# ferdean/lsa-fw

Measured on AMD Instinct MI355X. Metric: converged eigenpairs/sec (k=20, shift-invert), higher is better.
Workload: dtype c128

## Files before the change

lsa-fw_amd/csrc/ndlu.hip:

```cpp
#include <algorithm>
#include <chrono>
#include <cmath>
#include <cstdlib>
#include <functional>
#include <new>
#include <string>

#include "lsa_internal.h"
#include "nd_internal.h"

int k_allgather_inplace(lsa_ctx* ctx, void* vec, size_t bytes_per_rank);

namespace {

constexpr int kRT = 32;
constexpr int kCH = 1024;
constexpr int kGT = 64;

inline double now_s() { return std::chrono::duration<double>(std::chrono::steady_clock::now().time_since_epoch()).count(); }
inline size_t esize(int dtype) { return dtype == LSA_C128 ? 16 : 8; }

struct NdNodeDev {
    int64_t front_off;
    int64_t lfac_off;
// ... 1070 lines not shown
    for (int32_t c0 = 0; c0 < b; c0 += kCH) {
        const int32_t cn = min(kCH, b - c0);
        for (int32_t j = tid; j < cn; j += 256) vs[j] = bv[c0 + j];
        __syncthreads();
        if (c0 == 0) two_row_dot_prefetched<LPR>(Ua, Ub, vs, cn, sl, acc0, acc1, pa, pb);
        else two_row_dot<LPR>(Ua + c0, Ub + c0, vs, cn, sl, acc0, acc1);
        __syncthreads();
    }
    acc0 = lanes_sum<LPR>(acc0);
    acc1 = lanes_sum<LPR>(acc1);
    if (sl == 0) {
        if (ra < m) {
            const VT v = s_sub(xa, acc0);
            x[ia] = v;
            push_down(ge, nd.nchild, f, ra, xb, v);
        }
        if (rb < m) {
            const VT v = s_sub(xc, acc1);
            x[ib] = v;
            push_down(ge, nd.nchild, f, rb, xb, v);
        }
    }
    if (nd.nchild > 0) {
        const int32_t ntile = (m + ROWS - 1) / ROWS;
        const int64_t total = (int64_t)nd.nchild * b;
        for (int64_t e = (int64_t)ty * 256 + tid; e < total; e += (int64_t)ntile * 256) {
            const int32_t c = (int32_t)(e / b), j = (int32_t)(e - (int64_t)c * b);
            const int32_t g = ge[(size_t)c * f + m + j];
            if (g >= 0) xb[g] = bv[j];
        }
    }
}

template <typename MT, typename VT, int LPR, bool ORDERED>
__global__ __launch_bounds__(256) void nd_bwd_kernel(const NdSweepNode* __restrict__ lnodes, const MT* __restrict__ ufac,
                                                     const int32_t* __restrict__ idx, const int32_t* __restrict__ gell, VT* __restrict__ x,
                                                     VT* __restrict__ xb) {
    __shared__ VT vs[kCH];
    const NdSweepNode nd = lnodes[blockIdx.x];
    const int32_t r0 = (int32_t)blockIdx.y * (512 / LPR);
    if (r0 >= nd.m || nd.f == nd.m) return;
    nd_bwd_tile<MT, VT, LPR, ORDERED>(nd, r0, (int32_t)blockIdx.y, vs, ufac, idx, gell, x, xb);
}

constexpr int kNdBatchMax = 16;
struct NdBatchPtrs {
    const void* lfac[kNdBatchMax];
    const void* ufac[kNdBatchMax];
    const void* rhs[kNdBatchMax];
    void* x[kNdBatchMax];
    void* ubuf[kNdBatchMax];
    void* acc[kNdBatchMax];
    void* xb[kNdBatchMax];
};

template <typename MT, typename VT, int LPR, bool ORDERED>
__global__ __launch_bounds__(256) void nd_fwd_batch_kernel(const NdSweepNode* __restrict__ lnodes, const int32_t* __restrict__ idx,
                                                           const int32_t* __restrict__ gell, const int32_t* __restrict__ cmap, NdBatchPtrs p) {
    __shared__ VT vs[kCH];
    const NdSweepNode nd = lnodes[blockIdx.x];
    const int32_t r0 = (int32_t)blockIdx.y * (512 / LPR);
    if (r0 >= nd.orows + nd.brow) return;
    const int z = blockIdx.z;
    nd_fwd_tile<MT, VT, LPR, ORDERED>(nd, r0, vs, (const MT*)p.lfac[z], idx, gell, cmap, (const VT*)p.rhs[z], (VT*)p.x[z], (VT*)p.ubuf[z], (VT*)p.acc[z],
                                      (VT*)p.xb[z]);
}

template <typename MT, typename VT, int LPR, bool ORDERED>
__global__ __launch_bounds__(256) void nd_bwd_batch_kernel(const NdSweepNode* __restrict__ lnodes, const int32_t* __restrict__ idx,
                                                           const int32_t* __restrict__ gell, NdBatchPtrs p) {
    __shared__ VT vs[kCH];
    const NdSweepNode nd = lnodes[blockIdx.x];
    const int32_t r0 = (int32_t)blockIdx.y * (512 / LPR);
    if (r0 >= nd.m || nd.f == nd.m) return;
    const int z = blockIdx.z;
    nd_bwd_tile<MT, VT, LPR, ORDERED>(nd, r0, (int32_t)blockIdx.y, vs, (const MT*)p.ufac[z], idx, gell, (VT*)p.x[z], (VT*)p.xb[z]);
}

template <typename VT, bool ORDERED>
__global__ __launch_bounds__(256) void nd_dist_pack_kernel(const int32_t* __restrict__ dnodes, const NdNodeDev* __restrict__ nodes,
                                                           const int32_t* __restrict__ idx, int32_t rank, const VT* __restrict__ x, VT* __restrict__ xg) {
    const NdNodeDev nd = nodes[dnodes[blockIdx.x]];
    const int32_t r = (int32_t)blockIdx.y * 256 + threadIdx.x;
    if (r >= nd.orows) return;
    const int32_t j = nd.orow0 + r;
    xg[nd.xg_base + (int64_t)rank * nd.xg_stride + r] = x[ORDERED ? nd.own0 + j : idx[nd.idx_off + j]];
}

template <typename VT, bool ORDERED>
__global__ __launch_bounds__(256) void nd_dist_unpack_kernel(const int32_t* __restrict__ dnodes, const NdNodeDev* __restrict__ nodes,
                                                             const int32_t* __restrict__ child_ptr, const int32_t* __restrict__ child_idx,
                                                             const int32_t* __restrict__ cmap, const int32_t* __restrict__ idx, int32_t nranks,
                                                             VT* x, const VT* __restrict__ xg, VT* xb) {
    const int32_t t = dnodes[blockIdx.x];
    const NdNodeDev nd = nodes[t];
    const int32_t m = nd.m, b = nd.f - m;
    const int32_t ms = (m + nranks - 1) / nranks;
    const int32_t i = (int32_t)blockIdx.z * 256 + threadIdx.x;
    (void)b;
    auto own_val = [&](int32_t j) -> VT { return xg[nd.xg_base + (int64_t)(j / ms) * nd.xg_stride + j % ms]; };
    if (blockIdx.y == 0) {
        if (i >= m) return;
        x[ORDERED ? nd.own0 + i : idx[nd.idx_off + i]] = own_val(i);
        return;
    }
    const int32_t cp = child_ptr[t] + (int32_t)blockIdx.y - 1;
    if (cp >= child_ptr[t + 1]) return;
    const NdNodeDev nc = nodes[child_idx[cp]];
    if (i >= nc.f - nc.m) return;
    const int32_t p = cmap[nc.cmap_off + i];
    xb[nc.u_off + i] = p < m ? own_val(p) : xb[nd.u_off + (p - m)];
}

template <bool CONJ, typename MT>
__device__ __forceinline__ MT maybe_conj(MT a) {
    if constexpr (CONJ) return s_conj(a);
    else return a;
}

template <typename MT, typename VT, bool CONJ, bool DOWN>
__global__ __launch_bounds__(256) void nd_sweepT_kernel(const NdSweepNode* __restrict__ lnodes, const MT* __restrict__ lfac, const MT* __restrict__ ufac,
                                                        const int32_t* __restrict__ idx, const int32_t* __restrict__ gell,
                                                        const VT* __restrict__ rhs, VT* __restrict__ x, VT* __restrict__ ubuf,
                                                        const int64_t* __restrict__ tgoff, VT* __restrict__ pz, int64_t tg_slot, int32_t rank) {
    __shared__ VT vs[kCH];
    __shared__ VT part[4][64];
    const NdSweepNode nd = lnodes[blockIdx.x];
    const int32_t m = nd.m, f = nd.f, b = f - m;
    const bool dist = (nd.flags & 1) != 0;
// ... 62 lines not shown
        x[ix[r]] = s_add(x[ix[r]], z);
    } else if (r < m) {
        x[ix[r]] = z;
    } else {
        const int32_t j = r - m, w = (b + nranks - 1) / nranks, owner = j / w;
        const VT u = s_sub(gather_updates(gell + nd.ge_off, nd.nchild, f, r, ubuf, scalar_traits<VT>::zero()), z);
        ubuf[nd.u_off + (int64_t)(owner - rank) * ux_slot + (j - owner * w)] = u;
    }
}

}

struct lsa_ndlu {
    lsa_ctx* ctx = nullptr;
    NdSymbolic S;
    int dtype = LSA_C128;
    bool ordered = false;
    std::vector<NdChunk> chunks;
    std::vector<NdLevel> levels;
    NdNodeDev* d_nodes = nullptr;
    NdSweepNode *d_lnodes = nullptr, *d_lnodes_bwd = nullptr;
    int32_t *d_dist_nodes = nullptr, *d_child_ptr = nullptr, *d_child_idx = nullptr;
    void *d_xstage = nullptr, *d_xg = nullptr;
    int64_t* d_tgoff = nullptr;
    void* d_tg = nullptr;
    std::vector<int64_t> tg_slot;
    int64_t tg_slot_max = 0;
    int64_t xstage_slot = 0;
    std::vector<int64_t> h_upd_off, h_lfac_off;
    int64_t chunk_node_upd_off(int32_t t) const { return h_upd_off[(size_t)t]; }
    int32_t* d_gell = nullptr;
    int32_t *d_idx = nullptr, *d_cmap = nullptr, *d_tiles = nullptr, *d_chunk_nodes = nullptr;
    int64_t* d_asm_dst = nullptr;
    int32_t* d_asm_src = nullptr;
    int64_t asm_count = 0;
    int32_t *d_ipiv = nullptr, *d_rowq = nullptr, *d_flag = nullptr, *d_xflag = nullptr;
    unsigned long long* d_maxabs = nullptr;
    void *d_lfac = nullptr, *d_ufac = nullptr;
    void *d_work = nullptr, *d_upd = nullptr;
    void *d_ubuf = nullptr, *d_xb = nullptr, *d_acc = nullptr;
    void *d_tmp = nullptr, *d_ybuf = nullptr;
    int64_t lfac_entries = 0, ufac_entries = 0, work_entries = 0, upd_entries = 0, acc_entries = 0;
    int64_t xupd_slot = 0;
    int32_t *d_cand[2] = {nullptr, nullptr};
    void* d_dinv = nullptr;
    int32_t tp_min = 1 << 30;
    int32_t sb_min = 1 << 30;
    int32_t sb_cols = 128;
    int32_t ycap = 32;
    hipStream_t side = nullptr;
    hipEvent_t ev_panel = nullptr, ev_pivots = nullptr;
    double seconds_analyse = 0.0, seconds_numeric = 0.0;
    int32_t solve_launches = 0;
    int acc_vbytes = 0;
};

namespace {

void nd_free(lsa_ndlu* f) {
    if (!f) return;
    for (void* p : {(void*)f->d_lnodes_bwd, (void*)f->d_dist_nodes, (void*)f->d_child_ptr, (void*)f->d_child_idx, f->d_xstage, f->d_xg, (void*)f->d_tgoff, f->d_tg})
        if (p) (void)hipFree(p);
    for (void* p : {(void*)f->d_nodes, (void*)f->d_lnodes, (void*)f->d_gell, (void*)f->d_idx, (void*)f->d_cmap, (void*)f->d_tiles,
                    (void*)f->d_chunk_nodes, (void*)f->d_asm_dst, (void*)f->d_asm_src, (void*)f->d_ipiv, (void*)f->d_rowq, (void*)f->d_flag, (void*)f->d_xflag, (void*)f->d_maxabs,
                    f->d_lfac, f->d_ufac, f->d_work, f->d_upd, f->d_ubuf, f->d_xb, f->d_acc, f->d_tmp, f->d_ybuf, (void*)f->d_cand[0], (void*)f->d_cand[1], f->d_dinv})
        if (p) (void)hipFree(p);
    if (f->ev_panel) (void)hipEventDestroy(f->ev_panel);
    if (f->ev_pivots) (void)hipEventDestroy(f->ev_pivots);
    if (f->side) (void)hipStreamDestroy(f->side);
    delete f;
}

template <typename U>
int upload(lsa_ctx* ctx, const std::vector<U>& h, U** d) {
    const size_t bytes = std::max<size_t>(h.size(), 1) * sizeof(U);
    LSA_HIP_ALLOC(ctx, hipMalloc((void**)d, bytes));
    if (!h.empty()) LSA_HIP_CHECK(ctx, hipMemcpy(*d, h.data(), h.size() * sizeof(U), hipMemcpyHostToDevice));
    return LSA_OK;
}

int nd_setup(lsa_ctx* ctx, lsa_ndlu* f, int64_t free_agreed = 0) {
    NdSymbolic& S = f->S;
    const int32_t nt = S.nt;
    const size_t es = esize(f->dtype);
    const bool dist = S.nranks > 1;
    {
        const char* e = getenv("LSA_ND_TP_MIN");
        f->tp_min = e && *e ? std::max(1, atoi(e)) : 512;
        const char* sbm = getenv("LSA_ND_SB_MIN");
        f->sb_min = std::max(f->tp_min, sbm && *sbm ? std::max(1, atoi(sbm)) : 1024);
        f->ycap = kNB;
        const char* sbc = getenv("LSA_ND_SB_COLS");
        f->sb_cols = sbc && *sbc ? std::min(1024, std::max(kGT, atoi(sbc) / kGT * kGT)) : kSB;
    }
    LSA_HIP_ALLOC(ctx, hipMalloc((void**)&f->d_xflag, 4 * sizeof(int32_t) * (size_t)std::max(1, S.nranks)));
    f->ordered = true;
    for (size_t k = 0; k < S.perm.size() && f->ordered; ++k) f->ordered = S.perm[k] == (int32_t)k || dist;
    if (dist)
        for (int32_t t = 0; t < nt && f->ordered; ++t)
            for (int32_t r = 1; r < S.m[(size_t)t]; ++r)
                if (S.idx[(size_t)S.idx_off[(size_t)t] + r] != S.idx[(size_t)S.idx_off[(size_t)t]] + r) {
                    f->ordered = false;
                    break;
                }
    std::vector<NdNodeDev> nodes((size_t)nt);
    std::vector<int32_t> tiles;
    auto begin_list = [&](TileList& tl) { tl.off = (int64_t)tiles.size() / 2; tl.count = 0; };
    auto push = [&](TileList& tl, int32_t a, int32_t b) {
        tiles.push_back(a);
        tiles.push_back(b);
        ++tl.count;
    };
    int64_t budget = 0;
    {
        size_t free_b = 0, total_b = 0;
        if (hipMemGetInfo(&free_b, &total_b) != hipSuccess) free_b = (size_t)16 << 30;
        const int64_t after = (int64_t)free_b - S.factor_entries * (int64_t)es;
        budget = std::max<int64_t>(after / 4, (int64_t)256 << 20) / (int64_t)es;
        if (S.has_dist) budget = std::max<int64_t>((free_agreed > 0 ? free_agreed : (int64_t)free_b) / 6, (int64_t)256 << 20) / (int64_t)es;
        if (const char* e = getenv("LSA_ND_WORK_MB")) budget = std::max<int64_t>(atoll(e), 1) * (1 << 20) / (int64_t)es;
    }
    if (getenv("LSA_ND_TEST_OOM"))
        return lsa_set_error(ctx, LSA_ERR_OOM, "lsa_ndlu: out of device memory (forced by LSA_ND_TEST_OOM)");
    NdMemoryPlan P;
    nd_memory_plan(S, budget, P);
    for (int32_t t = 0; t < nt; ++t) {
        NdNodeDev& nd = nodes[(size_t)t];
        nd.front_off = P.work_off[(size_t)t];
        nd.lfac_off = P.lfac_off[(size_t)t];
        nd.ufac_off = P.ufac_off[(size_t)t];
// ... 236 lines not shown
                for (int32_t cp = S.child_ptr[(size_t)t]; cp < S.child_ptr[(size_t)t + 1]; ++cp) {
                    const int32_t ch = S.child_idx[(size_t)cp];
                    L.dist_rows = std::max(L.dist_rows, S.f[(size_t)ch] - S.m[(size_t)ch]);
                }
            }
        }
        LSA_CHECK(upload(ctx, lnodes, &f->d_lnodes));
        LSA_CHECK(upload(ctx, bnodes, &f->d_lnodes_bwd));
        LSA_CHECK(upload(ctx, dist_nodes, &f->d_dist_nodes));
        LSA_CHECK(upload(ctx, S.child_ptr, &f->d_child_ptr));
        LSA_CHECK(upload(ctx, S.child_idx, &f->d_child_idx));
        if (f->xstage_slot > 0) LSA_HIP_ALLOC(ctx, hipMalloc(&f->d_xstage, (size_t)f->xstage_slot * (size_t)S.nranks * es));
        if (S.xg_entries > 0) LSA_HIP_ALLOC(ctx, hipMalloc(&f->d_xg, (size_t)S.xg_entries * 16));
    }
    LSA_CHECK(upload(ctx, S.gell, &f->d_gell));
    LSA_CHECK(upload(ctx, S.idx, &f->d_idx));
    LSA_CHECK(upload(ctx, S.cmap, &f->d_cmap));
    LSA_CHECK(upload(ctx, chunk_nodes, &f->d_chunk_nodes));
    LSA_CHECK(upload(ctx, tiles, &f->d_tiles));
    const size_t nn = (size_t)std::max<int32_t>(S.n, 1);
    LSA_HIP_ALLOC(ctx, hipMalloc((void**)&f->d_ipiv, nn * sizeof(int32_t)));
    LSA_HIP_ALLOC(ctx, hipMalloc((void**)&f->d_rowq, nn * sizeof(int32_t)));
    LSA_HIP_ALLOC(ctx, hipMalloc((void**)&f->d_flag, 4 * sizeof(int32_t)));
    LSA_HIP_ALLOC(ctx, hipMalloc((void**)&f->d_maxabs, sizeof(unsigned long long)));
    LSA_HIP_ALLOC(ctx, hipMalloc(&f->d_lfac, (size_t)std::max<int64_t>(f->lfac_entries, 1) * es));
    LSA_HIP_ALLOC(ctx, hipMalloc(&f->d_ufac, (size_t)std::max<int64_t>(f->ufac_entries, 1) * es));
    LSA_HIP_ALLOC(ctx, hipMalloc(&f->d_work, (size_t)f->work_entries * es));
    LSA_HIP_ALLOC(ctx, hipMalloc(&f->d_upd, (size_t)f->upd_entries * es));
    const size_t ub = (size_t)std::max<int64_t>(S.u_off[(size_t)nt], 1) * 16;
    LSA_HIP_ALLOC(ctx, hipMalloc(&f->d_ubuf, ub));
    LSA_HIP_ALLOC(ctx, hipMalloc(&f->d_xb, ub));
    LSA_HIP_ALLOC(ctx, hipMalloc(&f->d_acc, (size_t)std::max<int64_t>(f->acc_entries, 1) * 16));
    LSA_HIP_CHECK(ctx, hipMemsetAsync(f->d_acc, 0, (size_t)std::max<int64_t>(f->acc_entries, 1) * 16, ctx->stream));
    LSA_HIP_CHECK(ctx, hipMemsetAsync(f->d_ubuf, 0, ub, ctx->stream));
    LSA_HIP_CHECK(ctx, hipMemsetAsync(f->d_xb, 0, ub, ctx->stream));
    LSA_HIP_ALLOC(ctx, hipMalloc(&f->d_tmp, nn * 16));
    LSA_HIP_ALLOC(ctx, hipMalloc(&f->d_ybuf, nn * (size_t)f->ycap * es));
    if (widest_tp > 0) {
        const size_t cand = ((size_t)S.n / kTRmin + (size_t)nt + 1) * kNB * sizeof(int32_t);
        LSA_HIP_ALLOC(ctx, hipMalloc((void**)&f->d_cand[0], cand));
        LSA_HIP_ALLOC(ctx, hipMalloc((void**)&f->d_cand[1], cand));
        LSA_HIP_ALLOC(ctx, hipMalloc(&f->d_dinv, (size_t)widest_tp * kNB * kNB * es));
        const char* la = getenv("LSA_ND_LOOKAHEAD");
        if (!(la && *la && atoi(la) == 0)) {
            int lo_pri = 0, hi_pri = 0;
            LSA_HIP_CHECK(ctx, hipDeviceGetStreamPriorityRange(&lo_pri, &hi_pri));
            LSA_HIP_CHECK(ctx, hipStreamCreateWithPriority(&f->side, hipStreamNonBlocking, hi_pri));
            LSA_HIP_CHECK(ctx, hipEventCreateWithFlags(&f->ev_panel, hipEventDisableTiming));
            LSA_HIP_CHECK(ctx, hipEventCreateWithFlags(&f->ev_pivots, hipEventDisableTiming));
        }
    }
    f->solve_launches = 0;
    for (const NdLevel& L : f->levels) f->solve_launches += (L.fwd_tiles > 0) + (L.bwd_tiles > 0);
    return LSA_OK;
}

template <typename T, int NT, int RPT, int W>
void launch_block(lsa_ctx* ctx, lsa_ndlu* f, const NdChunk& L, int32_t kb, double tiny2) {
    hipStream_t st = ctx->stream;
    const int32_t* lv = f->d_chunk_nodes + L.node_begin;
    T* front = (T*)f->d_work;
    auto active_at = [&](int32_t k) {
        return (int32_t)(std::lower_bound(L.sorted_m.begin(), L.sorted_m.end(), k, std::greater<int32_t>()) - L.sorted_m.begin());
    };
    const int32_t kend = std::min(kb + kNB, L.max_m);
    const bool others = std::min(kNB, L.max_m - kb) > W;
    int32_t kprev = -1, active_prev = 0;
    for (int32_t k0 = kb; k0 < kend; k0 += W) {
        const int32_t active = active_at(k0);
        if (active == 0) break;
        hipLaunchKernelGGL((nd_gj_fused_kernel<T, NT, RPT, W>), dim3(std::max(active, active_prev), others && kprev >= 0 ? 1 + kNB / 16 : 1), dim3(NT), 0, st, lv,
                           f->d_nodes, front, f->d_ipiv, f->d_rowq, kb, k0, kprev, f->d_flag, tiny2);
        kprev = k0;
        active_prev = active;
    }
    if (others && kprev >= 0)
        hipLaunchKernelGGL((nd_gj_fused_kernel<T, NT, RPT, W>), dim3(active_prev, 1 + kNB / 16), dim3(NT), 0, st, lv, f->d_nodes, front, f->d_ipiv, f->d_rowq, kb,
                           -1, kprev, f->d_flag, tiny2);
    if (L.max_m > kNB) {
        const int32_t active = active_at(kb);
        hipLaunchKernelGGL((nd_gj_stage_kernel<T>), dim3(active, (L.max_m + 255) / 256), dim3(256), 0, st, lv, f->d_nodes, (const T*)front, f->d_ipiv, kb,
                           kNB, kNB, 0, L.max_m, (T*)f->d_ybuf);
        const int32_t tiles = (L.max_m + kGT - 1) / kGT;
        hipLaunchKernelGGL((nd_gj_gemm_kernel<T>), dim3(active, tiles, tiles), dim3(256), 0, st, lv, f->d_nodes, front, f->d_rowq, kb, (const T*)f->d_ybuf, 0, 0,
                           0, 0, 0);
    }
}

template <typename T>
void launch_tournament(lsa_ndlu* f, const NdChunk& L, int32_t kb, double tiny2, hipStream_t st) {
    const int32_t* lv = f->d_chunk_nodes + L.node_begin;
    const T* front = (const T*)f->d_work;
    const int32_t active = (int32_t)(std::lower_bound(L.sorted_m.begin(), L.sorted_m.end(), kb, std::greater<int32_t>()) - L.sorted_m.begin());
    if (active == 0) return;
    int32_t sets = (L.max_m + tp_first<T>::rows - 1) / tp_first<T>::rows;
    hipLaunchKernelGGL((nd_tp_round_kernel<T, true, false>), dim3(active, sets), dim3(256), 0, st, lv, f->d_nodes, front, f->d_ipiv, f->d_rowq, kb, 0,
                       (const int32_t*)nullptr, f->d_cand[0], (T*)nullptr, f->d_flag, tiny2);
    int src = 0;
    for (int32_t round = 0;; ++round) {
        const int32_t groups = (sets + kTA - 1) / kTA;
        if (groups == 1) {
            hipLaunchKernelGGL((nd_tp_round_kernel<T, false, true>), dim3(active, 1), dim3(256), 0, st, lv, f->d_nodes, front, f->d_ipiv, f->d_rowq, kb, round,
                               (const int32_t*)f->d_cand[src], (int32_t*)nullptr, (T*)f->d_dinv, f->d_flag, tiny2);
            break;
        }
        hipLaunchKernelGGL((nd_tp_round_kernel<T, false, false>), dim3(active, groups), dim3(256), 0, st, lv, f->d_nodes, front, f->d_ipiv, f->d_rowq, kb, round,
// ... 106 lines not shown
        }
        for (const TileList& e : L.ext)
            if (e.count > 0)
                hipLaunchKernelGGL((nd_extend_add_kernel<T>), dim3(e.count), dim3(256), 0, st, tl + 2 * e.off, f->d_nodes, f->d_cmap, front, (const T*)upd);
        for (const auto& step : L.xsteps) {
            T* stage = (T*)f->d_xstage;
            int64_t stride = 0;
            for (int r = 0; r < S.nranks; ++r) {
                const NdChunk::XPiece& pc = step[(size_t)r];
                if (pc.nrows > 0) stride = std::max(stride, (int64_t)pc.nrows * (S.f[(size_t)pc.child] - S.m[(size_t)pc.child]));
            }
            if (stride == 0) continue;
            const NdChunk::XPiece& mine = step[(size_t)S.rank];
            if (mine.nrows > 0) {
                const int32_t bc = S.f[(size_t)mine.child] - S.m[(size_t)mine.child];
                const int64_t src_off = f->chunk_node_upd_off(mine.child) + (int64_t)(mine.row0 - S.brow0[(size_t)mine.child]) * bc;
                LSA_HIP_CHECK(ctx, hipMemcpyAsync(stage + (size_t)S.rank * (size_t)stride, upd + src_off, (size_t)mine.nrows * (size_t)bc * sizeof(T),
                                                  hipMemcpyDeviceToDevice, st));
            }
            LSA_CHECK(k_allgather_inplace(ctx, stage, (size_t)stride * sizeof(T)));
            for (int r = 0; r < S.nranks; ++r) {
                const NdChunk::XPiece& pc = step[(size_t)r];
                if (pc.nrows <= 0) continue;
                hipLaunchKernelGGL((nd_extend_add_staged_kernel<T>), dim3((pc.nrows + 15) / 16), dim3(256), 0, st, f->d_nodes, f->d_cmap, front,
                                   (const T*)(stage + (size_t)r * (size_t)stride), pc.child, pc.row0, pc.nrows);
            }
        }
        if (L.max_m >= f->tp_min) LSA_CHECK(launch_level_tp<T>(ctx, f, L, tiny2));
        for (int32_t kb = 0; kb < L.max_m && L.max_m < f->tp_min; kb += kNB) {
            if (L.max_m <= 64) launch_block<T, 64, 1, 8>(ctx, f, L, kb, tiny2);
            else if (L.max_m <= 128) launch_block<T, 128, 1, 8>(ctx, f, L, kb, tiny2);
            else if (L.max_m <= 256) launch_block<T, 256, 1, 8>(ctx, f, L, kb, tiny2);
            else if (L.max_m <= 512) launch_block<T, 512, 1, 8>(ctx, f, L, kb, tiny2);
            else if (L.max_m <= 1024) launch_block<T, 1024, 1, 8>(ctx, f, L, kb, tiny2);
            else if (L.max_m <= 2048) launch_block<T, 1024, 2, 8>(ctx, f, L, kb, tiny2);
            else if (L.max_m <= 4096) launch_block<T, 1024, 4, 4>(ctx, f, L, kb, tiny2);
            else if (L.max_m <= 8192) launch_block<T, 1024, 8, 2>(ctx, f, L, kb, tiny2);
            else launch_block<T, 1024, 16, 1>(ctx, f, L, kb, tiny2);
        }
        if (L.unperm.count > 0)
            hipLaunchKernelGGL((nd_unperm_kernel<T>), dim3(L.unperm.count), dim3(256), 0, st, tl + 2 * L.unperm.off, f->d_nodes, front, f->d_ipiv,
                               f->d_rowq, lfac);
        auto product = [&](auto kind) {
            constexpr int KIND = decltype(kind)::value;
            if (L.gemm[KIND].count == 0) return;
            hipLaunchKernelGGL((nd_gemm_mfma_kernel<T, KIND>), dim3(L.gemm[KIND].count), dim3(256), 0, st, tl + 2 * L.gemm[KIND].off, f->d_nodes, front, lfac, ufac);
        };
        product(std::integral_constant<int, 0>{});
        product(std::integral_constant<int, 1>{});
        product(std::integral_constant<int, 2>{});
        if (L.save.count > 0)
            hipLaunchKernelGGL((nd_save_update_kernel<T>), dim3(L.save.count), dim3(256), 0, st, tl + 2 * L.save.off, f->d_nodes, (const T*)front, upd);
    }
    if (!exchanged && S.nranks > 1 && f->xupd_slot > 0)
        LSA_CHECK(k_allgather_inplace(ctx, f->d_upd, (size_t)f->xupd_slot * sizeof(T)));
    int32_t hflag[4] = {0, 0, 0, 0};
    if (S.nranks > 1) {
        LSA_HIP_CHECK(ctx, hipMemcpyAsync(f->d_xflag + 4 * S.rank, f->d_flag, 4 * sizeof(int32_t), hipMemcpyDeviceToDevice, st));
        LSA_CHECK(k_allgather_inplace(ctx, f->d_xflag, 4 * sizeof(int32_t)));
        std::vector<int32_t> all((size_t)4 * S.nranks, 0);
        LSA_HIP_CHECK(ctx, hipMemcpyAsync(all.data(), f->d_xflag, all.size() * sizeof(int32_t), hipMemcpyDeviceToHost, st));
        LSA_HIP_CHECK(ctx, hipStreamSynchronize(st));
        for (int r = 0; r < S.nranks; ++r)
            if (all[(size_t)4 * r + 1] != 0) {
                memcpy(hflag, &all[(size_t)4 * r], sizeof hflag);
                if (r != S.rank) hflag[1] = -(r + 1);
                break;
            }
    } else {
        LSA_HIP_CHECK(ctx, hipMemcpyAsync(hflag, f->d_flag, sizeof hflag, hipMemcpyDeviceToHost, st));
        LSA_HIP_CHECK(ctx, hipStreamSynchronize(st));
    }
    LSA_HIP_CHECK(ctx, hipGetLastError());
    if (hflag[1] < 0)
        return lsa_set_error(ctx, LSA_ERR_ZERO_PIVOT, "lsa_ndlu: a pivot block on rank %d is singular to 1e-15 * max|C| (column %d of its node)", -hflag[1] - 1,
                             hflag[2]);
    if (hflag[1] != 0) {
        const int32_t t = hflag[1] - 1;
        const unsigned long long hi = (unsigned long long)(uint32_t)hflag[3] << 32;
        double mag2;
        memcpy(&mag2, &hi, sizeof mag2);
        return lsa_set_error(ctx, LSA_ERR_ZERO_PIVOT,
                             "lsa_ndlu: the pivot block of tree node %d (%d unknowns, front %d, level %d) is singular at its column %d: largest "
                             "candidate pivot %.3e against max|C| = %.3e (threshold 1e-15 max|C|); the matrix is singular, or needs pivoting "
                             "across fronts",
                             t, S.m[(size_t)t], S.f[(size_t)t], S.level[(size_t)t], hflag[2], std::sqrt(mag2), std::sqrt(max2));
    }
    if (const char* pe = getenv("LSA_ND_TEST_PERTURB")) {
        const double eps = atof(pe);
        if (eps != 0.0 && f->ufac_entries > 0) {
            const int blocks = (int)std::min<int64_t>((f->ufac_entries + 255) / 256, (int64_t)ctx->num_cu * 16);
            hipLaunchKernelGGL((nd_scale_kernel<T>), dim3(blocks), dim3(256), 0, st, f->ufac_entries, ufac, 1.0 + eps);
            LSA_HIP_CHECK(ctx, hipStreamSynchronize(st));
        }
    }
    return LSA_OK;
}

template <typename MT, typename VT, bool ORDERED>
int nd_apply_ordered(lsa_ctx* ctx, lsa_ndlu* f, const VT* b, VT* x) {
    hipStream_t st = ctx->stream;
    const MT* lfac = (const MT*)f->d_lfac;
    const MT* ufac = (const MT*)f->d_ufac;
    const NdSymbolic& S = f->S;
    VT *ubuf = (VT*)f->d_ubuf, *acc = (VT*)f->d_acc, *xb = (VT*)f->d_xb;
    if (f->acc_vbytes != (int)sizeof(VT)) {
        LSA_HIP_CHECK(ctx, hipMemsetAsync(f->d_acc, 0, (size_t)std::max<int64_t>(f->acc_entries, 1) * 16, st));
        f->acc_vbytes = (int)sizeof(VT);
    }
    for (size_t li = 0; li <= f->levels.size(); ++li) {
        if ((int32_t)li == S.phase_b_level && S.nranks > 1 && S.xu_slot > 0) LSA_CHECK(k_allgather_inplace(ctx, f->d_ubuf, (size_t)S.xu_slot * sizeof(VT)));
        if (li == f->levels.size()) break;
        const NdLevel& L = f->levels[li];
        if (L.fwd_tiles > 0) {
            const dim3 grid(L.node_count, L.fwd_tiles);
            const NdSweepNode* ln = f->d_lnodes + L.node_begin;
            if (L.sweep_rows == 8)
                hipLaunchKernelGGL((nd_fwd_kernel<MT, VT, 64, ORDERED>), grid, dim3(256), 0, st, ln, lfac, f->d_idx, f->d_gell, f->d_cmap, b, x, ubuf, acc, xb);
            else if (L.sweep_rows == 128)
                hipLaunchKernelGGL((nd_fwd_kernel<MT, VT, 4, ORDERED>), grid, dim3(256), 0, st, ln, lfac, f->d_idx, f->d_gell, f->d_cmap, b, x, ubuf, acc, xb);
            else
                hipLaunchKernelGGL((nd_fwd_kernel<MT, VT, 16, ORDERED>), grid, dim3(256), 0, st, ln, lfac, f->d_idx, f->d_gell, f->d_cmap, b, x, ubuf, acc, xb);
        }
        if (L.dist_count > 0 && L.ux_slot > 0) LSA_CHECK(k_allgather_inplace(ctx, ubuf + L.ux_base, (size_t)L.ux_slot * sizeof(VT)));
    }
    for (size_t l = f->levels.size(); l-- > 0;) {
        const NdLevel& L = f->levels[l];
        if (L.bwd_tiles > 0) {
            const dim3 grid(L.node_count, L.bwd_tiles);
            const NdSweepNode* ln = f->d_lnodes_bwd + L.node_begin;
            if (L.sweep_rows == 8) hipLaunchKernelGGL((nd_bwd_kernel<MT, VT, 64, ORDERED>), grid, dim3(256), 0, st, ln, ufac, f->d_idx, f->d_gell, x, xb);
            else hipLaunchKernelGGL((nd_bwd_kernel<MT, VT, 16, ORDERED>), grid, dim3(256), 0, st, ln, ufac, f->d_idx, f->d_gell, x, xb);
        }
        if (L.dist_count > 0) {
            const int32_t* dn = f->d_dist_nodes + L.dist_begin;
            VT* xg = (VT*)f->d_xg;
            if (L.xg_slot > 0) {
                hipLaunchKernelGGL((nd_dist_pack_kernel<VT, ORDERED>), dim3(L.dist_count, (L.dist_rows + 255) / 256), dim3(256), 0, st, dn, f->d_nodes, f->d_idx, S.rank,
                                   (const VT*)x, xg);
                LSA_CHECK(k_allgather_inplace(ctx, xg + L.xg_base, (size_t)L.xg_slot * sizeof(VT)));
            }
            hipLaunchKernelGGL((nd_dist_unpack_kernel<VT, ORDERED>), dim3(L.dist_count, 1 + L.dist_children, (L.dist_rows + 255) / 256), dim3(256), 0, st, dn, f->d_nodes,
                               f->d_child_ptr, f->d_child_idx, f->d_cmap, f->d_idx, S.nranks, x, (const VT*)xg, xb);
        }
    }
    LSA_HIP_CHECK(ctx, hipGetLastError());
    return LSA_OK;
}

template <typename MT, typename VT>
int nd_apply(lsa_ctx* ctx, lsa_ndlu* f, const VT* b, VT* x) {
    return f->ordered ? nd_apply_ordered<MT, VT, true>(ctx, f, b, x) : nd_apply_ordered<MT, VT, false>(ctx, f, b, x);
}

template <typename MT, typename VT, bool ORDERED>
int nd_apply_batch_ordered(lsa_ctx* ctx, int32_t J, lsa_ndlu* const* f, const VT* const* b, VT* const* x) {
    hipStream_t st = ctx->stream;
    const lsa_ndlu* f0 = f[0];
    NdBatchPtrs p;
    memset(&p, 0, sizeof p);
    for (int32_t z = 0; z < J; ++z) {
        if (f[z]->acc_vbytes != (int)sizeof(VT)) {
            LSA_HIP_CHECK(ctx, hipMemsetAsync(f[z]->d_acc, 0, (size_t)std::max<int64_t>(f[z]->acc_entries, 1) * 16, st));
            f[z]->acc_vbytes = (int)sizeof(VT);
        }
        p.lfac[z] = f[z]->d_lfac;
        p.ufac[z] = f[z]->d_ufac;
        p.rhs[z] = b[z];
        p.x[z] = x[z];
        p.ubuf[z] = f[z]->d_ubuf;
        p.acc[z] = f[z]->d_acc;
        p.xb[z] = f[z]->d_xb;
    }
    for (const NdLevel& L : f0->levels) {
        if (L.fwd_tiles == 0) continue;
        const dim3 grid(L.node_count, L.fwd_tiles, J);
        const NdSweepNode* ln = f0->d_lnodes + L.node_begin;
        if (L.sweep_rows == 8)
            hipLaunchKernelGGL((nd_fwd_batch_kernel<MT, VT, 64, ORDERED>), grid, dim3(256), 0, st, ln, f0->d_idx, f0->d_gell, f0->d_cmap, p);
        else if (L.sweep_rows == 128)
            hipLaunchKernelGGL((nd_fwd_batch_kernel<MT, VT, 4, ORDERED>), grid, dim3(256), 0, st, ln, f0->d_idx, f0->d_gell, f0->d_cmap, p);
        else
            hipLaunchKernelGGL((nd_fwd_batch_kernel<MT, VT, 16, ORDERED>), grid, dim3(256), 0, st, ln, f0->d_idx, f0->d_gell, f0->d_cmap, p);
    }
    for (size_t l = f0->levels.size(); l-- > 0;) {
        const NdLevel& L = f0->levels[l];
        if (L.bwd_tiles == 0) continue;
        const dim3 grid(L.node_count, L.bwd_tiles, J);
        const NdSweepNode* ln = f0->d_lnodes_bwd + L.node_begin;
        if (L.sweep_rows == 8) hipLaunchKernelGGL((nd_bwd_batch_kernel<MT, VT, 64, ORDERED>), grid, dim3(256), 0, st, ln, f0->d_idx, f0->d_gell, p);
        else hipLaunchKernelGGL((nd_bwd_batch_kernel<MT, VT, 16, ORDERED>), grid, dim3(256), 0, st, ln, f0->d_idx, f0->d_gell, p);
    }
    LSA_HIP_CHECK(ctx, hipGetLastError());
    return LSA_OK;
}

template <typename MT, typename VT>
int nd_apply_batch(lsa_ctx* ctx, int32_t J, lsa_ndlu* const* f, const VT* const* b, VT* const* x) {
    return f[0]->ordered ? nd_apply_batch_ordered<MT, VT, true>(ctx, J, f, b, x) : nd_apply_batch_ordered<MT, VT, false>(ctx, J, f, b, x);
}

bool nd_batch_compatible(const lsa_ndlu* f, const lsa_ndlu* g) {
    const NdSymbolic &A = f->S, &B = g->S;
    if (A.nranks != 1 || B.nranks != 1 || A.has_dist || B.has_dist) return false;
    if (f->dtype != g->dtype || f->ordered != g->ordered || A.n != B.n || A.nnz != B.nnz || A.pattern_hash != B.pattern_hash ||
        A.constraint_hash != B.constraint_hash || A.tree_hash != B.tree_hash || A.leaf_size != B.leaf_size)
        return false;
    if (f->lfac_entries != g->lfac_entries || f->ufac_entries != g->ufac_entries || f->acc_entries != g->acc_entries || f->h_lfac_off != g->h_lfac_off ||
        f->h_upd_off != g->h_upd_off || A.lvl_nodes != B.lvl_nodes || f->levels.size() != g->levels.size())
        return false;
    for (size_t l = 0; l < f->levels.size(); ++l) {
        const NdLevel &a = f->levels[l], &c = g->levels[l];
        if (a.node_begin != c.node_begin || a.node_count != c.node_count || a.fwd_tiles != c.fwd_tiles || a.bwd_tiles != c.bwd_tiles ||
            a.sweep_rows != c.sweep_rows || a.dist_count != 0 || c.dist_count != 0)
            return false;
    }
    return true;
}

}

namespace {
int nd_ensure_transposed_dist(lsa_ctx* ctx, lsa_ndlu* f) {
    const NdSymbolic& S = f->S;
    if (!S.has_dist || f->d_tgoff) return LSA_OK;
    std::vector<int64_t> off(S.lvl_nodes.size(), -1);
    f->tg_slot.assign(f->levels.size(), 0);
    f->tg_slot_max = 0;
    for (size_t l = 0; l < f->levels.size(); ++l) {
        const NdLevel& L = f->levels[l];
        int64_t run = 0;
        for (int32_t q = 0; q < L.node_count; ++q) {
            const int32_t t = S.lvl_nodes[(size_t)L.node_begin + q];
            if (S.kind[(size_t)t] != 4) continue;
            off[(size_t)L.node_begin + q] = run;
            run += S.f[(size_t)t];
        }
        f->tg_slot[l] = run;
        f->tg_slot_max = std::max(f->tg_slot_max, run);
    }
    LSA_HIP_ALLOC(ctx, hipMalloc(&f->d_tg, (size_t)std::max<int64_t>(f->tg_slot_max, 1) * (size_t)S.nranks * 16));
    LSA_CHECK(upload(ctx, off, &f->d_tgoff));
    return LSA_OK;
}

template <typename MT, typename VT, bool CONJ>
int nd_apply_T(lsa_ctx* ctx, lsa_ndlu* f, const VT* b, VT* x) {
    hipStream_t st = ctx->stream;
    const MT* lfac = (const MT*)f->d_lfac;
    const MT* ufac = (const MT*)f->d_ufac;
    const NdSymbolic& S = f->S;
    LSA_CHECK(nd_ensure_transposed_dist(ctx, f));
    VT* pz = (VT*)f->d_tg;
    for (size_t li = 0; li <= f->levels.size(); ++li) {
        if ((int32_t)li == S.phase_b_level && S.nranks > 1 && S.xu_slot > 0) LSA_CHECK(k_allgather_inplace(ctx, f->d_ubuf, (size_t)S.xu_slot * sizeof(VT)));
        if (li == f->levels.size()) break;
        const NdLevel& L = f->levels[li];
        const int64_t slot = L.dist_count > 0 ? f->tg_slot[li] : 0;
        if (L.fwd_tiles > 0)
            hipLaunchKernelGGL((nd_sweepT_kernel<MT, VT, CONJ, false>), dim3(L.node_count, (L.max_f + 63) / 64), dim3(256), 0, st, f->d_lnodes + L.node_begin,
                               lfac, ufac, f->d_idx, f->d_gell, b, x, (VT*)f->d_ubuf, f->d_tgoff ? f->d_tgoff + L.node_begin : nullptr, pz, slot, S.rank);
        if (L.dist_count > 0) {
            LSA_CHECK(k_allgather_inplace(ctx, pz, (size_t)slot * sizeof(VT)));
            hipLaunchKernelGGL((nd_distT_finish_kernel<VT, false>), dim3(L.node_count, (L.max_f + 255) / 256), dim3(256), 0, st, f->d_lnodes + L.node_begin,
                               f->d_tgoff + L.node_begin, f->d_idx, f->d_gell, (const VT*)pz, slot, S.nranks, S.rank, L.ux_slot, x, (VT*)f->d_ubuf);
        }
    }
    for (size_t l = f->levels.size(); l-- > 0;) {
        const NdLevel& L = f->levels[l];
// ... 350 lines not shown
    LSA_HIP_CHECK(ctx, hipStreamSynchronize(ctx->stream));
    return LSA_OK;
}

int lsa_ndlu_solve_time(lsa_ctx* ctx, lsa_ndlu* f, const lsa_vec* b, lsa_vec* x, int iters, double* avg_ms) {
    if (!ctx || !f || !b || !x || !avg_ms || iters < 1) return lsa_set_error(ctx, LSA_ERR_ARG, "lsa_ndlu_solve_time: bad argument");
    if (b->n != f->S.n || x->n != f->S.n || b->dtype != x->dtype || b->d == x->d) return lsa_set_error(ctx, LSA_ERR_ARG, "lsa_ndlu_solve_time: shape/dtype mismatch");
    LSA_HIP_CHECK(ctx, hipEventRecord(ctx->ev0, ctx->stream));
    for (int i = 0; i < iters; ++i) LSA_CHECK(ndlu_solve_dev(ctx, f, b->dtype, b->d, x->d));
    LSA_HIP_CHECK(ctx, hipEventRecord(ctx->ev1, ctx->stream));
    LSA_HIP_CHECK(ctx, hipEventSynchronize(ctx->ev1));
    float ms = 0.f;
    LSA_HIP_CHECK(ctx, hipEventElapsedTime(&ms, ctx->ev0, ctx->ev1));
    *avg_ms = (double)ms / iters;
    return LSA_OK;
}

int lsa_ndlu_inertia(lsa_ctx* ctx, lsa_ndlu* f, int64_t* negative, int64_t* zero, int64_t* positive) {
    if (!ctx || !f || !negative || !zero || !positive) return lsa_set_error(ctx, LSA_ERR_ARG, "lsa_ndlu_inertia: null argument");
    if (f->dtype != LSA_F64) return lsa_set_error(ctx, LSA_ERR_ARG, "lsa_ndlu_inertia: needs real factors (a real symmetric matrix)");
    if (f->S.nranks != 1) return lsa_set_error(ctx, LSA_ERR_ARG, "lsa_ndlu_inertia: not available for a forest cut over ranks");
    *negative = *zero = *positive = 0;
    const NdSymbolic& S = f->S;
    std::vector<double> blk;
    LSA_HIP_CHECK(ctx, hipStreamSynchronize(ctx->stream));
    for (int32_t t = 0; t < S.nt; ++t) {
        const int32_t m = S.m[(size_t)t];
        if (m <= 0) continue;
        blk.resize((size_t)m * m);
        LSA_HIP_CHECK(ctx, hipMemcpy(blk.data(), (const double*)f->d_lfac + f->h_lfac_off[(size_t)t], (size_t)m * m * sizeof(double), hipMemcpyDeviceToHost));
        int64_t ng = 0, ze = 0, ps = 0;
        const int rc = lsa_dense_sym_inertia(m, blk.data(), m, 1e-13, &ng, &ze, &ps);
        if (rc != LSA_OK) return lsa_set_error(ctx, rc, "lsa_ndlu_inertia: the pivot block of tree node %d holds non-finite values", t);
        *negative += ng;
        *zero += ze;
        *positive += ps;
    }
    return LSA_OK;
}

int lsa_ndlu_info(const lsa_ndlu* f, int32_t* ntree, int32_t* nlevels, int32_t* max_front, int64_t* factor_entries, int64_t* front_entries,
                  int64_t* apply_bytes, int32_t* apply_launches, double* seconds_analyse, double* seconds_numeric) {
    if (!f) return LSA_ERR_ARG;
    const NdSymbolic& S = f->S;
    if (ntree) *ntree = S.nt;
    if (nlevels) *nlevels = S.nlevels;
    if (max_front) {
        int32_t mf = 0;
        for (int32_t v : S.f) mf = std::max(mf, v);
        *max_front = mf;
    }
    if (factor_entries) *factor_entries = S.factor_entries;
    if (front_entries) *front_entries = f->lfac_entries + f->ufac_entries + f->work_entries + f->upd_entries;
    if (apply_bytes) *apply_bytes = S.factor_entries * (int64_t)esize(f->dtype) + 16 * (3 * (int64_t)S.n + 2 * S.u_off[(size_t)S.nt]);
    if (apply_launches) *apply_launches = f->solve_launches;
    if (seconds_analyse) *seconds_analyse = f->seconds_analyse;
    if (seconds_numeric) *seconds_numeric = f->seconds_numeric;
    return LSA_OK;
}

}
```

Measured before the change: 536.4.

## Replace top two ND levels of triangular solve with explicit inverse matvec

After numeric factorization, builds an explicit dense inverse of the combined root-plus-children block (up to 1280 rows) with a set of small GEMM jobs. The apply path then skips the sweep over the last two tree levels in both forward and backward passes and replaces them with a single dense matrix-vector kernel. This cuts serialized, low-parallelism kernel launches at the narrow top of the tree, which dominate each shift-invert solve. In exchange it adds extra factorization work and memory for the s×s block, and relies on the inverse being assembled correctly from the L/U factors.

Result: faster. 552.5, median of 6 (+3.0%).

```diff
diff --git a/lsa-fw_amd/csrc/ndlu.hip b/lsa-fw_amd/csrc/ndlu.hip
--- a/lsa-fw_amd/csrc/ndlu.hip
+++ b/lsa-fw_amd/csrc/ndlu.hip
@@ -1146,6 +1146,7 @@
     void* ubuf[kNdBatchMax];
     void* acc[kNdBatchMax];
     void* xb[kNdBatchMax];
+    const void* top[kNdBatchMax];
 };
 
 template <typename MT, typename VT, int LPR, bool ORDERED>
@@ -1169,6 +1170,152 @@
     if (r0 >= nd.m || nd.f == nd.m) return;
     const int z = blockIdx.z;
     nd_bwd_tile<MT, VT, LPR, ORDERED>(nd, r0, (int32_t)blockIdx.y, vs, (const MT*)p.ufac[z], idx, gell, (VT*)p.x[z], (VT*)p.xb[z]);
+}
+
+constexpr int kTopChildren = 8;
+struct NdTopNode {
+    int64_t acc_off, ge_off;
+    int32_t own0, m, f, nchild;
+    int32_t off, pad0;
+};
+struct NdTop {
+    int32_t s, nchild;
+    NdTopNode node[kTopChildren + 1];
+};
+
+struct NdTopJob {
+    int64_t a_off, b_off, c_off, d_off;
+    int32_t M, N, K, lda, ldb, ldd;
+    int32_t a_src, gather;
+    int32_t map_off, negate;
+};
+static_assert(sizeof(NdTopJob) == 72, "assembly job layout");
+
+template <typename T>
+__global__ __launch_bounds__(256) void nd_top_gemm_kernel(const int32_t* __restrict__ tiles, const NdTopJob* __restrict__ jobs,
+                                                          const int32_t* __restrict__ cmap, const T* __restrict__ lfac,
+                                                          const T* __restrict__ ufac, T* top, int32_t ldc) {
+    __shared__ T As[16][33], Bs[16][33];
+    const NdTopJob jb = jobs[tiles[2 * blockIdx.x]];
+    const int32_t tile = tiles[2 * blockIdx.x + 1], i0 = (tile >> 16) * 32, j0 = (tile & 0xFFFF) * 32;
+    const T* A = (jb.a_src == 0 ? lfac : jb.a_src == 1 ? ufac : (const T*)top) + jb.a_off;
+    const T* B = lfac + jb.b_off;
+    const int32_t* map = cmap + jb.map_off;
+    const int tid = threadIdx.x, ti = tid / 16, tj = tid % 16;
+    T acc[2][2] = {{scalar_traits<T>::zero(), scalar_traits<T>::zero()}, {scalar_traits<T>::zero(), scalar_traits<T>::zero()}};
+    for (int32_t k0 = 0; k0 < jb.K; k0 += 16) {
+#pragma unroll
+        for (int h = 0; h < 2; ++h) {
+            const int32_t i = i0 + ti + 16 * h, k = k0 + tj;
+            As[tj][ti + 16 * h] = i < jb.M && k < jb.K ? A[(size_t)i * jb.lda + (jb.gather == 1 ? map[k] : k)] : scalar_traits<T>::zero();
+            const int32_t kb = k0 + tid / 32 + 8 * h, j = j0 + tid % 32;
+            Bs[tid / 32 + 8 * h][tid % 32] = kb < jb.K && j < jb.N ? B[(size_t)(jb.gather == 2 ? map[kb] : kb) * jb.ldb + j] : scalar_traits<T>::zero();
+        }
+        __syncthreads();
+#pragma unroll
+        for (int k = 0; k < 16; ++k) {
+            const T a0 = As[k][ti], a1 = As[k][ti + 16], b0 = Bs[k][tj], b1 = Bs[k][tj + 16];
+            fma_acc(acc[0][0], a0, b0);
+            fma_acc(acc[0][1], a0, b1);
+            fma_acc(acc[1][0], a1, b0);
+            fma_acc(acc[1][1], a1, b1);
+        }
+        __syncthreads();
+    }
+#pragma unroll
+    for (int h = 0; h < 2; ++h)
+#pragma unroll
+        for (int g = 0; g < 2; ++g) {
+            const int32_t i = i0 + ti + 16 * h, j = j0 + tj + 16 * g;
+            if (i >= jb.M || j >= jb.N) continue;
+            const T d = jb.d_off >= 0 ? lfac[jb.d_off + (size_t)i * jb.ldd + j] : scalar_traits<T>::zero();
+            top[jb.c_off + (size_t)i * ldc + j] = jb.negate ? s_sub(d, acc[h][g]) : s_add(d, acc[h][g]);
+        }
+}
+
+template <typename VT>
+__device__ __forceinline__ void nd_top_store(const NdTop& tp, int32_t i, VT val, const int32_t* __restrict__ icmap, const int32_t* __restrict__ gell,
+                                             VT* __restrict__ x, VT* __restrict__ xb) {
+    const int32_t K = tp.nchild;
+    const NdTopNode& R = tp.node[K];
+    if (i >= R.off) {
+        const int32_t k = i - R.off;
+        x[R.own0 + k] = val;
+        for (int32_t c = 0; c < K; ++c) {
+            const NdTopNode& nd = tp.node[c];
+            const int32_t p = icmap[(size_t)c * R.m + k];
+            if (p >= 0) push_down(gell + nd.ge_off, nd.nchild, nd.f, nd.m + p, xb, val);
+        }
+        return;
+    }
+    for (int32_t c = 0; c < K; ++c) {
+        const NdTopNode& nd = tp.node[c];
+        if (i < nd.off || i >= nd.off + nd.m) continue;
+        x[nd.own0 + i - nd.off] = val;
+        push_down(gell + nd.ge_off, nd.nchild, nd.f, i - nd.off, xb, val);
+    }
+}
+
+template <typename MT, typename VT>
+__device__ __forceinline__ void nd_top_tile(const NdTop& tp, int32_t r0, VT* vs, const MT* __restrict__ top, const int32_t* __restrict__ icmap,
+                                            const int32_t* __restrict__ gell, const VT* __restrict__ rhs, VT* __restrict__ x,
+                                            const VT* __restrict__ acc, VT* __restrict__ xb) {
+    constexpr int LPR = 64;
+    const int32_t s = tp.s, K = tp.nchild;
+    const NdTopNode& R = tp.node[K];
+    const int tid = threadIdx.x, sw = tid / LPR, sl = tid % LPR;
+    const int32_t ra = r0 + sw, rb = ra + 256 / LPR;
+    const MT* Ta = top + (size_t)min(ra, s - 1) * s;
+    const MT* Tb = top + (size_t)min(rb, s - 1) * s;
+    VT acc0 = scalar_traits<VT>::zero(), acc1 = scalar_traits<VT>::zero();
+    MT pa[4], pb[4];
+    row_pair_prefetch<LPR>(Ta, Tb, min(kCH, s), sl, pa, pb);
+    for (int32_t c0 = 0; c0 < s; c0 += kCH) {
+        const int32_t c1 = min(c0 + kCH, s);
+        for (int32_t c = 0; c < K; ++c) {
+            const NdTopNode& nd = tp.node[c];
+            const VT* slots = acc + nd.acc_off;
+            for (int32_t j = max(c0, nd.off) + tid; j < min(c1, nd.off + nd.m); j += 256) {
+                const int32_t r = j - nd.off;
+                vs[j - c0] = slot_sum(slots, nd.nchild, nd.f, r, rhs[nd.own0 + r]);
+            }
+        }
+        for (int32_t j = max(c0, R.off) + tid; j < c1; j += 256) {
+            const int32_t k = j - R.off;
+            VT z = rhs[R.own0 + k];
+            for (int32_t c = 0; c < K; ++c) {
+                const NdTopNode& nd = tp.node[c];
+                const int32_t p = icmap[(size_t)c * R.m + k];
+                if (p >= 0) z = s_add(z, slot_sum(acc + nd.acc_off, nd.nchild, nd.f, nd.m + p, scalar_traits<VT>::zero()));
+            }
+            vs[j - c0] = z;
+        }
+        __syncthreads();
+        if (c0 == 0) two_row_dot_prefetched<LPR>(Ta, Tb, vs, c1 - c0, sl, acc0, acc1, pa, pb);
+        else two_row_dot<LPR>(Ta + c0, Tb + c0, vs, c1 - c0, sl, acc0, acc1);
+        __syncthreads();
+    }
+    const VT s0 = lanes_sum<LPR>(acc0), s1 = lanes_sum<LPR>(acc1);
+    if (sl == 0) {
+        if (ra < s) nd_top_store(tp, ra, s0, icmap, gell, x, xb);
+        if (rb < s) nd_top_store(tp, rb, s1, icmap, gell, x, xb);
+    }
+}
+
+template <typename MT, typename VT>
+__global__ __launch_bounds__(256) void nd_top_kernel(NdTop tp, const MT* __restrict__ top, const int32_t* __restrict__ icmap,
+                                                     const int32_t* __restrict__ gell, const VT* __restrict__ rhs, VT* __restrict__ x,
+                                                     const VT* __restrict__ acc, VT* __restrict__ xb) {
+    __shared__ VT vs[kCH];
+    nd_top_tile<MT, VT>(tp, (int32_t)blockIdx.x * 8, vs, top, icmap, gell, rhs, x, acc, xb);
+}
+
+template <typename MT, typename VT>
+__global__ __launch_bounds__(256) void nd_top_batch_kernel(NdTop tp, const int32_t* __restrict__ icmap, const int32_t* __restrict__ gell, NdBatchPtrs p) {
+    __shared__ VT vs[kCH];
+    const int z = blockIdx.y;
+    nd_top_tile<MT, VT>(tp, (int32_t)blockIdx.x * 8, vs, (const MT*)p.top[z], icmap, gell, (const VT*)p.rhs[z], (VT*)p.x[z], (const VT*)p.acc[z],
+                        (VT*)p.xb[z]);
 }
 
 template <typename VT, bool ORDERED>
@@ -1337,6 +1484,14 @@
     hipEvent_t ev_panel = nullptr, ev_pivots = nullptr;
     double seconds_analyse = 0.0, seconds_numeric = 0.0;
     int32_t solve_launches = 0;
+    NdTop top = {};
+    int32_t top_level = -1;
+    void* d_top = nullptr;
+    int32_t* d_top_icmap = nullptr;
+    NdTopJob* d_top_jobs = nullptr;
+    int32_t* d_top_tiles = nullptr;
+    int32_t top_tiles[2] = {0, 0};
+    int64_t top_replaced_entries = 0;
     int acc_vbytes = 0;
 };
 
@@ -1344,6 +1499,8 @@
 
 void nd_free(lsa_ndlu* f) {
     if (!f) return;
+    for (void* p : {f->d_top, (void*)f->d_top_icmap, (void*)f->d_top_jobs, (void*)f->d_top_tiles})
+        if (p) (void)hipFree(p);
     for (void* p : {(void*)f->d_lnodes_bwd, (void*)f->d_dist_nodes, (void*)f->d_child_ptr, (void*)f->d_child_idx, f->d_xstage, f->d_xg, (void*)f->d_tgoff, f->d_tg})
         if (p) (void)hipFree(p);
     for (void* p : {(void*)f->d_nodes, (void*)f->d_lnodes, (void*)f->d_gell, (void*)f->d_idx, (void*)f->d_cmap, (void*)f->d_tiles,
@@ -1361,6 +1518,85 @@
     const size_t bytes = std::max<size_t>(h.size(), 1) * sizeof(U);
     LSA_HIP_ALLOC(ctx, hipMalloc((void**)d, bytes));
     if (!h.empty()) LSA_HIP_CHECK(ctx, hipMemcpy(*d, h.data(), h.size() * sizeof(U), hipMemcpyHostToDevice));
+    return LSA_OK;
+}
+
+int nd_setup_top(lsa_ctx* ctx, lsa_ndlu* f, const std::vector<NdNodeDev>& nodes) {
+    const NdSymbolic& S = f->S;
+    f->top = NdTop{};
+    f->top_level = -1;
+    static const int32_t limit = getenv("LSA_ND_TOPINV") && *getenv("LSA_ND_TOPINV") ? std::max(0, atoi(getenv("LSA_ND_TOPINV"))) : 1280;
+    if (limit <= 0 || S.nranks != 1 || S.has_dist || !f->ordered || S.nlevels < 3) return LSA_OK;
+    const int32_t lr = S.nlevels - 1;
+    if (S.lvl_ptr[(size_t)lr + 1] - S.lvl_ptr[(size_t)lr] != 1) return LSA_OK;
+    const int32_t R = S.lvl_nodes[(size_t)S.lvl_ptr[(size_t)lr]];
+    int32_t roots = 0;
+    for (int32_t t = 0; t < S.nt; ++t) roots += S.parent[(size_t)t] < 0;
+    const int32_t c0 = S.child_ptr[(size_t)R], K = S.child_ptr[(size_t)R + 1] - c0, mR = S.m[(size_t)R];
+    if (roots != 1 || S.parent[(size_t)R] >= 0 || S.f[(size_t)R] != mR || K < 1 || K > kTopChildren) return LSA_OK;
+    if (S.lvl_ptr[(size_t)lr] - S.lvl_ptr[(size_t)lr - 1] != K) return LSA_OK;
+    NdTop tp = {};
+    tp.nchild = K;
+    int64_t s = 0, replaced = (int64_t)mR * mR;
+    for (int32_t ci = 0; ci < K; ++ci) {
+        const int32_t c = S.child_idx[(size_t)c0 + ci];
+        const NdNodeDev& nd = nodes[(size_t)c];
+        bool on_level = false;
+        for (int32_t q = S.lvl_ptr[(size_t)lr - 1]; q < S.lvl_ptr[(size_t)lr]; ++q) on_level |= S.lvl_nodes[(size_t)q] == c;
+        if (!on_level || nd.nchild < 1 || nd.acc_off < 0 || nd.f <= nd.m || nd.m < 1 || S.kind[(size_t)c] == 3 || S.kind[(size_t)c] == 4) return LSA_OK;
+        tp.node[ci] = NdTopNode{nd.acc_off, nd.ge_off, nd.own0, nd.m, nd.f, nd.nchild, (int32_t)s, 0};
+        s += nd.m;
+        replaced += (int64_t)nd.m * nd.m + 2 * (int64_t)nd.m * (nd.f - nd.m);
+    }
+    const NdNodeDev& nr = nodes[(size_t)R];
+    tp.node[K] = NdTopNode{nr.acc_off, nr.ge_off, nr.own0, mR, mR, K, (int32_t)s, 0};
+    s += mR;
+    if (s > limit) return LSA_OK;
+    tp.s = (int32_t)s;
+    std::vector<int32_t> icmap((size_t)K * mR, -1);
+    for (int32_t ci = 0; ci < K; ++ci) {
+        const int32_t c = S.child_idx[(size_t)c0 + ci];
+        for (int32_t p = 0; p < S.f[(size_t)c] - S.m[(size_t)c]; ++p) {
+            const int32_t k = S.cmap[(size_t)S.cmap_off[(size_t)c] + p];
+            if (k < 0 || k >= mR) return LSA_OK;
+            icmap[(size_t)ci * mR + k] = p;
+        }
+    }
+    std::vector<NdTopJob> jobs;
+    std::vector<int32_t> tiles;
+    auto add = [&](const NdTopJob& jb) {
+        for (int32_t ti = 0; ti < (jb.M + 31) / 32; ++ti)
+            for (int32_t tj = 0; tj < (jb.N + 31) / 32; ++tj) {
+                tiles.push_back((int32_t)jobs.size());
+                tiles.push_back((ti << 16) | tj);
+            }
+        jobs.push_back(jb);
+    };
+    const int64_t oR = tp.node[K].off;
+    add(NdTopJob{0, 0, oR * s + oR, nr.lfac_off, mR, mR, 0, 1, 1, mR, 0, 0, 0, 0});
+    for (int32_t ci = 0; ci < K; ++ci) {
+        const NdNodeDev& nd = nodes[(size_t)S.child_idx[(size_t)c0 + ci]];
+        const int32_t m = nd.m, b = nd.f - nd.m;
+        const int64_t o = tp.node[ci].off;
+        add(NdTopJob{nd.ufac_off, nr.lfac_off, o * s + oR, -1, m, mR, b, b, mR, 0, 1, 2, nd.cmap_off, 1});
+        add(NdTopJob{nr.lfac_off, nd.lfac_off + (int64_t)m * m, oR * s + o, -1, mR, m, b, mR, m, 0, 0, 1, nd.cmap_off, 0});
+    }
+    f->top_tiles[0] = (int32_t)tiles.size() / 2;
+    for (int32_t ci = 0; ci < K; ++ci)
+        for (int32_t di = 0; di < K; ++di) {
+            const NdNodeDev &nc = nodes[(size_t)S.child_idx[(size_t)c0 + ci]], &nd = nodes[(size_t)S.child_idx[(size_t)c0 + di]];
+            add(NdTopJob{tp.node[ci].off * s + oR, nd.lfac_off + (int64_t)nd.m * nd.m, tp.node[ci].off * s + tp.node[di].off, ci == di ? nc.lfac_off : -1, nc.m,
+                         nd.m, nd.f - nd.m, (int32_t)s, nd.m, nc.m, 2, 1, nd.cmap_off, 0});
+        }
+    f->top_tiles[1] = (int32_t)tiles.size() / 2 - f->top_tiles[0];
+    LSA_CHECK(upload(ctx, icmap, &f->d_top_icmap));
+    LSA_CHECK(upload(ctx, jobs, &f->d_top_jobs));
+    LSA_CHECK(upload(ctx, tiles, &f->d_top_tiles));
+    LSA_HIP_ALLOC(ctx, hipMalloc(&f->d_top, (size_t)(s * s) * esize(f->dtype)));
+    f->top = tp;
+    f->top_level = lr;
+    f->top_replaced_entries = replaced;
+    f->solve_launches -= 2;
     return LSA_OK;
 }
 
@@ -1703,6 +1939,7 @@
     }
     f->solve_launches = 0;
     for (const NdLevel& L : f->levels) f->solve_launches += (L.fwd_tiles > 0) + (L.bwd_tiles > 0);
+    LSA_CHECK(nd_setup_top(ctx, f, nodes));
     return LSA_OK;
 }
 
@@ -1915,6 +2152,11 @@
         if (L.save.count > 0)
             hipLaunchKernelGGL((nd_save_update_kernel<T>), dim3(L.save.count), dim3(256), 0, st, tl + 2 * L.save.off, f->d_nodes, (const T*)front, upd);
     }
+    if (f->top.s > 0)
+        for (int q = 0, t0 = 0; q < 2; t0 += f->top_tiles[q++])
+            if (f->top_tiles[q] > 0)
+                hipLaunchKernelGGL((nd_top_gemm_kernel<T>), dim3(f->top_tiles[q]), dim3(256), 0, st, f->d_top_tiles + 2 * t0, f->d_top_jobs, f->d_cmap,
+                                   (const T*)lfac, (const T*)ufac, (T*)f->d_top, f->top.s);
     if (!exchanged && S.nranks > 1 && f->xupd_slot > 0)
         LSA_CHECK(k_allgather_inplace(ctx, f->d_upd, (size_t)f->xupd_slot * sizeof(T)));
     int32_t hflag[4] = {0, 0, 0, 0};
@@ -1967,6 +2209,7 @@
     const MT* ufac = (const MT*)f->d_ufac;
     const NdSymbolic& S = f->S;
     VT *ubuf = (VT*)f->d_ubuf, *acc = (VT*)f->d_acc, *xb = (VT*)f->d_xb;
+    const bool top = f->top.s > 0;
     if (f->acc_vbytes != (int)sizeof(VT)) {
         LSA_HIP_CHECK(ctx, hipMemsetAsync(f->d_acc, 0, (size_t)std::max<int64_t>(f->acc_entries, 1) * 16, st));
         f->acc_vbytes = (int)sizeof(VT);
@@ -1975,7 +2218,11 @@
         if ((int32_t)li == S.phase_b_level && S.nranks > 1 && S.xu_slot > 0) LSA_CHECK(k_allgather_inplace(ctx, f->d_ubuf, (size_t)S.xu_slot * sizeof(VT)));
         if (li == f->levels.size()) break;
         const NdLevel& L = f->levels[li];
-        if (L.fwd_tiles > 0) {
+        if (ORDERED && top && (int32_t)li + 1 == f->top_level) continue;
+        if (ORDERED && top && (int32_t)li == f->top_level) {
+            hipLaunchKernelGGL((nd_top_kernel<MT, VT>), dim3((f->top.s + 7) / 8), dim3(256), 0, st, f->top, (const MT*)f->d_top, f->d_top_icmap, f->d_gell, b, x,
+                               (const VT*)acc, xb);
+        } else if (L.fwd_tiles > 0) {
             const dim3 grid(L.node_count, L.fwd_tiles);
             const NdSweepNode* ln = f->d_lnodes + L.node_begin;
             if (L.sweep_rows == 8)
@@ -1989,7 +2236,7 @@
     }
     for (size_t l = f->levels.size(); l-- > 0;) {
         const NdLevel& L = f->levels[l];
-        if (L.bwd_tiles > 0) {
+        if (L.bwd_tiles > 0 && !(ORDERED && top && (int32_t)l + 1 == f->top_level)) {
             const dim3 grid(L.node_count, L.bwd_tiles);
             const NdSweepNode* ln = f->d_lnodes_bwd + L.node_begin;
             if (L.sweep_rows == 8) hipLaunchKernelGGL((nd_bwd_kernel<MT, VT, 64, ORDERED>), grid, dim3(256), 0, st, ln, ufac, f->d_idx, f->d_gell, x, xb);
@@ -2034,8 +2281,16 @@
         p.ubuf[z] = f[z]->d_ubuf;
         p.acc[z] = f[z]->d_acc;
         p.xb[z] = f[z]->d_xb;
-    }
-    for (const NdLevel& L : f0->levels) {
+        p.top[z] = f[z]->d_top;
+    }
+    const bool top = ORDERED && f0->top.s > 0;
+    for (size_t li = 0; li < f0->levels.size(); ++li) {
+        const NdLevel& L = f0->levels[li];
+        if (top && (int32_t)li + 1 == f0->top_level) continue;
+        if (top && (int32_t)li == f0->top_level) {
+            hipLaunchKernelGGL((nd_top_batch_kernel<MT, VT>), dim3((f0->top.s + 7) / 8, J), dim3(256), 0, st, f0->top, f0->d_top_icmap, f0->d_gell, p);
+            continue;
+        }
         if (L.fwd_tiles == 0) continue;
         const dim3 grid(L.node_count, L.fwd_tiles, J);
         const NdSweepNode* ln = f0->d_lnodes + L.node_begin;
@@ -2048,7 +2303,7 @@
     }
     for (size_t l = f0->levels.size(); l-- > 0;) {
         const NdLevel& L = f0->levels[l];
-        if (L.bwd_tiles == 0) continue;
+        if (L.bwd_tiles == 0 || (top && (int32_t)l + 1 == f0->top_level)) continue;
         const dim3 grid(L.node_count, L.bwd_tiles, J);
         const NdSweepNode* ln = f0->d_lnodes_bwd + L.node_begin;
         if (L.sweep_rows == 8) hipLaunchKernelGGL((nd_bwd_batch_kernel<MT, VT, 64, ORDERED>), grid, dim3(256), 0, st, ln, f0->d_idx, f0->d_gell, p);
@@ -2078,6 +2333,7 @@
             a.sweep_rows != c.sweep_rows || a.dist_count != 0 || c.dist_count != 0)
             return false;
     }
+    if (f->top.s != g->top.s || f->top_level != g->top_level) return false;
     return true;
 }
 
@@ -2534,7 +2790,8 @@
     }
     if (factor_entries) *factor_entries = S.factor_entries;
     if (front_entries) *front_entries = f->lfac_entries + f->ufac_entries + f->work_entries + f->upd_entries;
-    if (apply_bytes) *apply_bytes = S.factor_entries * (int64_t)esize(f->dtype) + 16 * (3 * (int64_t)S.n + 2 * S.u_off[(size_t)S.nt]);
+    const int64_t swept = S.factor_entries - f->top_replaced_entries * (f->top.s > 0) + (int64_t)f->top.s * f->top.s;
+    if (apply_bytes) *apply_bytes = swept * (int64_t)esize(f->dtype) + 16 * (3 * (int64_t)S.n + 2 * S.u_off[(size_t)S.nt]);
     if (apply_launches) *apply_launches = f->solve_launches;
     if (seconds_analyse) *seconds_analyse = f->seconds_analyse;
     if (seconds_numeric) *seconds_numeric = f->seconds_numeric;
```
